# atom501/v-img

Measured on AMD Instinct MI355X. Metric: Mrays/sec (primary+secondary) at 512 spp, higher is better.
Workload: dtype f32; 1 GPU; disney_spheres.json, mis integrator, 512 spp, 1800x800; integrator=mis, spp=512, depth=unbounded, bvh=sweep SAH (host)

## Files before the change

v-img_amd/csrc/device_scene.h:

```cpp
#pragma once
#include <hip/hip_runtime.h>
#include <stdint.h>

#include "../../include/vimg_scene.h"
#include "material_record.h"

namespace vimg {

#define VIMG_GLOBAL __attribute__((address_space(1)))
#define VIMG_LDS __attribute__((address_space(3)))
template <typename T>
using gptr = const VIMG_GLOBAL T*;
typedef float v4f __attribute__((ext_vector_type(4)));
typedef uint32_t v2u __attribute__((ext_vector_type(2)));
typedef uint32_t v4u __attribute__((ext_vector_type(4)));

struct __attribute__((aligned(16))) DNode {
  v4f a;
  v4f b;
  v4f c;
  uint32_t left_ref, right_ref, pad0, pad1;
};
static_assert(sizeof(DNode) == 64, "DNode must be one 64-byte line");

// ... 61 lines not shown
};

struct RenderArgs {
  uint32_t integrator, samples, depth;
  uint32_t tile_rank, tile_world;
  uint32_t tiles_x, tiles_y;
  uint32_t num_local_tiles;
  uint32_t full_stats;
  uint32_t stack_entries;
  uint32_t lds_nodes;
  uint32_t stack_lds;
  VIMG_GLOBAL uint32_t* stack_ovf;
  VIMG_GLOBAL v4u* pool_cold;
  uint32_t lds_leaf;
  VIMG_GLOBAL v4u* pool_state;
  uint32_t pool_segments;
  uint32_t pool_seg_len;
  uint32_t pool_epoch;
  uint32_t pool_slots;
  uint32_t pool_refill;
  uint32_t pool_vbatch;
  uint32_t pool_boxmin;
  uint32_t pool_starve;
  uint32_t pool_gbreak;
  uint32_t pool_classes;
  uint32_t cu_walkers;
  uint32_t cu_flex;
  uint32_t cu_lowwater;
  uint32_t cu_patience;
  uint32_t cu_join;
  uint32_t cu_sleep;
  uint32_t cu_watchdog;
  uint32_t cu_magic_v, cu_shift_v;
  uint32_t cu_magic_w, cu_shift_w;
  int32_t single_x, single_y;
  uint32_t sample_base;
  float spp_div;
  const VIMG_GLOBAL v4u* prog_in;
  VIMG_GLOBAL v4u* prog_out;
  const VIMG_GLOBAL uint32_t* item_list;
  uint32_t item_count;
};

struct DeviceStats {
  unsigned long long closest, shadow, internal, leaf, prim, sphere, nan_samples;
  unsigned long long trip_descend, trip_prim, iterations;
  unsigned long long prof[28];
  unsigned long long wait_cyc[5], wait_n[5];
  unsigned long long px_done[3];
  unsigned long long px_hops[3];
  unsigned long long ray_cyc[2];
  unsigned long long pv_cyc[7];
  unsigned long long walk_cyc[4];
};

}
```

v-img_amd/csrc/render_cu_kernel.h:

```cpp
#pragma once
#include <type_traits>

#include "plain_build.h"
#include "render_kernels.h"

namespace vimg {

enum : uint32_t {
  SC_THROUGHPUT = 0,
  SC_RESULT,
  SC_NEE,
  SC4_RNG,
  SC4_MAIN
};
__host__ __device__ constexpr uint32_t cu_cold_records(bool tex) { return SC4_MAIN + 1u + (tex ? 1u : 0u); }
__host__ __device__ constexpr uint32_t cu_stack_rows_of(uint32_t entries, uint32_t in_lds) { return in_lds < entries ? in_lds + 1u : entries; }
constexpr uint32_t SLOT_IDLE = 0xffffffffu;

VD void state_store(VIMG_GLOBAL uint32_t* p, uint32_t v) {
  __hip_atomic_store(p, v, __ATOMIC_RELAXED, __HIP_MEMORY_SCOPE_AGENT);
}
VD uint32_t state_load(VIMG_GLOBAL uint32_t* p) {
  return __hip_atomic_load(p, __ATOMIC_RELAXED, __HIP_MEMORY_SCOPE_AGENT);
}
VD uint32_t lane_rank(unsigned long long mask, uint32_t lane) {
  return __popcll(mask & ((1ull << lane) - 1ull));
}

enum : uint32_t {
  CF_PRIMARY = 1u, CF_NONSPEC = 2u, CF_HAS_S = 4u, CF_HAS_R = 8u, CF_OCCLUDED = 16u, CF_FOUND = 32u,
  CF_FRESH = 64u, CF_KIND_SPHERE = 128u, CF_DONE_S = 256u, CF_DONE_R = 512u,
  CF_CLS_SHIFT = 10u,
  CF_DONE_V = 4096u,
  CF_KILL_R = 8192u,
  CF_BOUNCE_SHIFT = 16u
};
enum : uint32_t {
  CR_ORG = 0,
  CR_DIR,
  CR_SHD,
  CR_HIT,
  CR_COUNT
};
constexpr uint32_t CU_EMPTY = 0xffffu;
constexpr uint32_t CU_RAY_S = 0x8000u;
constexpr uint32_t CQ_WALK = 4u, CQ_COUNT = 5u;
constexpr uint32_t CU_LDS_BYTES = CR_COUNT * 16u + 8u + 4u * 2u + 2u * 2u + 4u;

struct CuCtl {
  int32_t avail[8];
  uint32_t tail[CQ_COUNT], head[CQ_COUNT];
  uint32_t live;
  uint32_t pixels_left;
  uint32_t abort;
  uint32_t t0_lo, t0_hi;
  uint32_t pad[1];
};
static_assert(sizeof(CuCtl) == 96, "CuCtl layout");
struct CuWaveRec {
  unsigned long long cyc[6], nbatch[4], nslots[4];
  uint32_t internal, leaf, prim, sphere;
  unsigned long long box_pass, box_lanes, leaf_round, leaf_lanes, sessions, refills, refill_rays, pad;
  unsigned long long looks, q_sum[4];
  unsigned long long w_cyc[4];
  unsigned long long wait_cyc[5], wait_n[5];
  unsigned long long ray_cyc, ray_n;
  unsigned long long pv_cyc[6], pv_n;
};
static_assert(sizeof(CuWaveRec) == 416, "CuWaveRec layout");
__host__ __device__ constexpr uint32_t cu_pool_bytes(uint32_t slots, uint32_t waves) {
  return CU_LDS_BYTES * slots + uint32_t(sizeof(CuCtl)) + waves * uint32_t(sizeof(CuWaveRec));
}
VD uint32_t cu_mod(uint32_t n, uint32_t d, uint32_t magic, uint32_t shift) { return n - d * (__umulhi(n, magic) >> shift); }
VD int32_t lds_add_rtn(VIMG_LDS int32_t* p, int32_t v) { return __hip_atomic_fetch_add(p, v, __ATOMIC_RELAXED, __HIP_MEMORY_SCOPE_WORKGROUP); }
VD uint32_t lds_add_rtn(VIMG_LDS uint32_t* p, uint32_t v) { return __hip_atomic_fetch_add(p, v, __ATOMIC_RELAXED, __HIP_MEMORY_SCOPE_WORKGROUP); }
VD uint32_t lds_load(VIMG_LDS uint32_t* p) { return __hip_atomic_load(p, __ATOMIC_RELAXED, __HIP_MEMORY_SCOPE_WORKGROUP); }
VD int32_t lds_load(VIMG_LDS int32_t* p) { return __hip_atomic_load(p, __ATOMIC_RELAXED, __HIP_MEMORY_SCOPE_WORKGROUP); }
VD uint32_t cu_uni(uint32_t v) { return static_cast<uint32_t>(__builtin_amdgcn_readfirstlane(static_cast<int>(v))); }

static_assert(PLAIN_INTEGRATOR_MIS == uint32_t(VIMG_INTEGRATOR_MIS), "plain_build.h");
template <uint32_t PLAIN> VD uint32_t opt_integrator(const RenderArgs& A) {
  if constexpr (PLAIN & PF_INTEGRATOR) return uint32_t(VIMG_INTEGRATOR_MIS); else return A.integrator;
}
template <uint32_t PLAIN> VD uint32_t opt_classes(const RenderArgs& A) {
  if constexpr (PLAIN & PF_CLASSES) return 3u; else return A.pool_classes;
}
template <uint32_t PLAIN> VD bool opt_leaf_in_lds(const RenderArgs& A) {
  if constexpr (PLAIN & PF_LEAF_LDS) return true; else return A.lds_leaf != 0u;
}
template <uint32_t PLAIN> VD bool opt_single(const RenderArgs& A) {
  if constexpr (PLAIN & PF_SINGLE) return false; else return A.single_x >= 0;
}
template <uint32_t PLAIN> VD bool opt_has_items(const RenderArgs& A) {
  if constexpr (PLAIN & PF_ITEMS) return false; else return A.item_list != nullptr;
}
template <uint32_t PLAIN> VD uint32_t opt_flex(const RenderArgs& A) {
  if constexpr (PLAIN & PF_FLEX) return PLAIN_FLEX_DEFAULT; else return A.cu_flex;
}


struct CuKArgs {
  DScene g;
  RenderArgs A;
  float* out;
  DeviceStats* stats;
  unsigned int* work_counter;
};
typedef const __attribute__((address_space(4))) CuKArgs* CuKPtr;
VD CuKPtr cu_kargs() {
  unsigned long long p = reinterpret_cast<unsigned long long>(__builtin_amdgcn_kernarg_segment_ptr());
  asm volatile("" : "+s"(p));
  return (CuKPtr)p;
}

#define CU_STAGE_LOCALS(K)                                                                                              \
  extern __shared__ __attribute__((aligned(16))) unsigned char lds_raw[];                                               \
  [[maybe_unused]] const DScene& g = *(const DScene*)&(K)->g;                                                           \
  [[maybe_unused]] const RenderArgs& A = *(const RenderArgs*)&(K)->A;                                                   \
  [[maybe_unused]] float* __restrict__ out = (K)->out;                                                                  \
  [[maybe_unused]] unsigned int* __restrict__ work_counter = (K)->work_counter;                                         \
// ... 133 lines not shown
        VIMG_LDS uint16_t* e_ = ring_at(q, h_ + r_);                                                                    \
        uint32_t v_ = __hip_atomic_load(e_, __ATOMIC_RELAXED, __HIP_MEMORY_SCOPE_WORKGROUP), spins_ = 0;                \
        while (v_ == CU_EMPTY && !stuck_) {                                                                             \
          __builtin_amdgcn_s_sleep(1);                                                                                  \
          v_ = __hip_atomic_load(e_, __ATOMIC_RELAXED, __HIP_MEMORY_SCOPE_WORKGROUP);                                   \
          if (++spins_ > (1u << 22)) stuck_ = true;                                                                     \
        }                                                                                                               \
        __hip_atomic_store(e_, static_cast<uint16_t>(CU_EMPTY), __ATOMIC_RELAXED, __HIP_MEMORY_SCOPE_WORKGROUP);        \
        entry = v_;                                                                                                     \
      }                                                                                                                 \
    }                                                                                                                   \
    if (__any(stuck_)) {                                                                                                \
      if (lane == 0) raise(4u);                                                                                         \
      return 0u;                                                                                                        \
    }                                                                                                                   \
    return got_;                                                                                                        \
  }

template <bool TEX, int NW, bool DIAG, int EARLY, bool FIN, int MTC, uint32_t PLAIN>
VD void cu_vertex(uint32_t n, uint32_t slot, bool& all_pending, uint32_t& n_nan, uint32_t& n_dead) {
  const CuKPtr K = cu_kargs();
  CU_STAGE_LOCALS(K);
  constexpr bool finisher_batch = FIN;
  constexpr bool CAN_SPLIT = !FIN && MTC != int(VIMG_MAT_LAMBERTIAN);
  const bool split = CAN_SPLIT && n <= 32u && !(opt_flex<PLAIN>(A) & 16u);
  const bool mirror = split && lane >= 32u;
  if (split) slot = static_cast<uint32_t>(__shfl(static_cast<int>(slot), static_cast<int>(lane & 31u)));
  const bool on = (split ? (lane & 31u) : lane) < n;
  if (!on) slot = 0u;
  const v4u r_ray = on ? rd(CR_DIR, slot) : v4u{0u, 0u, 0u, 0u};
  uint32_t flags = r_ray.w;
  const bool fresh = on && (flags & CF_FRESH);
  const bool have = on && !fresh;
  uint32_t px = 0, py = 0, smp = 0, item = 0, bounce = 0;
  Rng rng{0};
  f3 acc{0.f, 0.f, 0.f}, ray_o{0.f, 0.f, 0.f}, ray_d{0.f, 0.f, 1.f};
  f3 throughput{1.f, 1.f, 1.f}, result{0.f, 0.f, 0.f};
  RayCone cone{0.f, 0.f};
  float eta_scale = 1.f, prev_pdf = 0.f;
  bool primary = true, non_specular_bounce = false;
  v4u r_origin{0u, 0u, 0u, 0u}, r_hit{0u, 0u, 0u, 0u}, r_nee{0u, 0u, 0u, 0u};
  v2u r_hx{0u, 0u};
  constexpr bool PV = DIAG && MTC == int(VIMG_MAT_PRINCIPLED);
  [[maybe_unused]] unsigned long long pv_t = PV ? __builtin_readcyclecounter() : 0ull;
  [[maybe_unused]] auto pv_lap = [&](int k) {
    if constexpr (PV) {
      if (full_stats) {
        const unsigned long long now = __builtin_readcyclecounter();
        if (lane == 0) wrec->pv_cyc[k] += now - pv_t;
        pv_t = now;
      }
    }
  };
  uint32_t hops = 0;
  if (full_stats && have) hops = recw[(CR_SHD * P + slot) * 4u + 3u] + 1u;
  if (have) {
    const v4u r_t = crd(SC_THROUGHPUT, slot), r_r = crd(SC_RESULT, slot);
    v4u r_a{0u, 0u, 0u, 0u};
    if (finisher_batch) r_a = cold_acc[slot];
    if (r_ray.w & CF_HAS_S) r_nee = crd(SC_NEE, slot);
    r_origin = rd(CR_ORG, slot);
    r_hit = rd(CR_HIT, slot);
    r_hx = hitx[slot];
    const v4u r_g = crd(SC4_RNG, slot);
    px = r_g.z & 0xffffu, py = r_g.z >> 16;
    smp = r_g.w;
    item = r_a.w;
    rng.s = uint64_t(r_g.x) | (uint64_t(r_g.y) << 32);
    acc = f3{uf(r_a.x), uf(r_a.y), uf(r_a.z)};
    ray_o = f3{uf(r_origin.x), uf(r_origin.y), uf(r_origin.z)};
    ray_d = f3{uf(r_ray.x), uf(r_ray.y), uf(r_ray.z)};
    throughput = f3{uf(r_t.x), uf(r_t.y), uf(r_t.z)};
    result = f3{uf(r_r.x), uf(r_r.y), uf(r_r.z)};
    eta_scale = uf(r_t.w);
    prev_pdf = uf(r_r.w);
    bounce = flags >> CF_BOUNCE_SHIFT;
    primary = (flags & CF_PRIMARY) != 0;
    non_specular_bounce = (flags & CF_NONSPEC) != 0;
    if constexpr (TEX) {
      const v4u r_c = cold_cone[slot];
      cone = RayCone{uf(r_c.x), uf(r_c.y)};
    }
  }

  pv_lap(0);
  bool finish = false, at_vertex = false;
  Hit hit;
  hit.p = f3{0.f, 0.f, 0.f};
  if (have) {
    if ((flags & CF_HAS_S) && !(flags & CF_OCCLUDED))
      result = result + f3{uf(r_nee.x), uf(r_nee.y), uf(r_nee.z)};
    if (!(flags & CF_HAS_R) || (flags & CF_KILL_R)) {
      finish = true;
    } else {
      const bool hit_any = (flags & CF_FOUND) != 0;
      if (hit_any) {
        HitRec hr;
        hr.e0 = uf(r_hit.x), hr.e1 = uf(r_hit.y), hr.e2 = uf(r_hit.z);
        hr.inv_det = uf(r_hit.w);
        hr.prim = r_hx.x;
        hr.kind = (flags & CF_KIND_SPHERE) ? 1u : 0u;
        TravRay tr{ray_o, ray_d, 0.0001f, uf(r_hx.y)};
        make_hit_info<TEX>(g, hr, tr, hit);
      }
      if (material_mode) {
        if (!hit_any) {
          result = throughput * background_emit<TEX>(g, ray_d, cone);
          finish = true;
        } else {
          at_vertex = true;
// ... 22 lines not shown
            at_vertex = true;
          }
        }
      } else {
        if (hit_any) {
          gptr<VimgMaterial> m = g.materials + hit.mat;
          if (m->type == VIMG_MAT_DIFFUSE_LIGHT) {
            const f3 le = mat_emitted(m, ray_d, hit.ns);
            if (prev_pdf != 0) {
              float light_pdf = surf_pdf(g, hit.prim, ray_o, hit.p, ray_d) / g.num_lights;
              float Gt = geometric_term(ray_o, hit.p, hit.ng);
              float mis_weight = balance_heuristic(prev_pdf * Gt, light_pdf);
              result = result + throughput * mis_weight * le;
            } else {
              result = result + throughput * le;
            }
            finish = true;
          } else {
            bool survive = true;
            if (bounce > roulette_threshold) {
              float rr = static_cast<float>(pcg_next(rng)) / 4294967296.0f;
              f3 rr_t = (1.f / eta_scale) * throughput;
              float max_val = sel_min(sel_max(sel_max(rr_t.x, rr_t.y), rr_t.z), 0.95f);
              if (rr > max_val)
                survive = false;
              else
                throughput = throughput / max_val;
            }
            if (survive) {
              bounce += 1;
              at_vertex = true;
            } else {
              finish = true;
            }
          }
        } else {
          if (prev_pdf != 0 && g.background_emissive) {
            float light_pdf = background_pdf<TEX>(g, ray_d) / g.num_lights;
            float mis_weight = balance_heuristic(prev_pdf, light_pdf);
            result = result + throughput * mis_weight * background_emit<TEX>(g, ray_d, cone);
          }
          finish = true;
        }
      }
      if (at_vertex && !(bounce < A.depth)) {
        at_vertex = false;
        finish = true;
      }
    }
  }

  pv_lap(1);
  if constexpr (!finisher_batch) {
    if (have && !mirror) {
      VIMG_GLOBAL uint32_t* rw = reinterpret_cast<VIMG_GLOBAL uint32_t*>(cold + (slot * SC4_MAIN + SC_RESULT));
      rw[0] = fu(result.x), rw[1] = fu(result.y), rw[2] = fu(result.z);
    }
  }
  bool has_s = false, has_r = false;
  bool early = false, pushed_r = false;
  bool rec_written = false;
  f3 shadow_d{0.f, 0.f, 1.f}, nee_contrib{0.f, 0.f, 0.f};
  float shadow_max_t = 0.f;
  if constexpr (!finisher_batch) {
    if (material_mode && at_vertex) {
      gptr<VimgMaterial> m = g.materials + hit.mat;
      const f3 emitted_col = mat_emitted(m, ray_d, hit.ns);
      Scatter sc = sample_mat<TEX>(g, hit, ray_d, rng, non_specular_bounce);
      if (!sc.valid) {
        result = throughput * emitted_col;
        finish = true;
      } else {
        if (!sc.is_specular) non_specular_bounce = true;
        if constexpr (TEX) {
          const float hd = length(ray_o - hit.p);
          const float ssa = spread_angle_from_curvature(hit.curvature, cone.cone_width, ray_d, hit.ns);
          if (sc.eta != 0.f)
            cone = propagate_refract_cone(cone, ray_d, ssa, sc.eta, sc.wo);
          else
            cone = propagate_reflect_cone(cone, ssa * 2.f, hd);
        }
        if (sc.eta != 0.f) eta_scale /= (sc.eta * sc.eta);
        f3 fdiv{0.f, 0.f, 0.f};
        const uint32_t type = m->type;
        if (type == VIMG_MAT_LAMBERTIAN) {
          fdiv = col_at_ray_hit<TEX>(g, m->tex, ray_d, cone, hit);
        } else if (type == VIMG_MAT_DIELECTRIC) {
          fdiv = splat3(1.f);
        } else if (type == VIMG_MAT_PRINCIPLED) {
          f3 f;
          float pdf;
          principled_eval_pdf<TEX>(g, m, ray_d, sc.wo, hit, cone, non_specular_bounce, f, pdf);
          fdiv = f / pdf;
        }
        throughput = throughput * (emitted_col + fdiv);
        bool survive = true;
        if (bounce > roulette_threshold) {
          float rr = static_cast<float>(pcg_next(rng)) / 4294967296.0f;
          f3 rr_t = (1.f / eta_scale) * throughput;
          float max_val = sel_min(sel_max(sel_max(rr_t.x, rr_t.y), rr_t.z), 0.95f);
          if (rr > max_val)
            survive = false;
          else
            throughput = throughput / max_val;
        }
        bounce += 1;
// ... 204 lines not shown
          }
          if (!valid) {
            have_claim = false;
          } else if (seg == 0u) {
            if (A.sample_base == 0u) {
              const uint64_t image_index = uint64_t(px) + uint64_t(H - 1 - py) * W;
              pcg_seed(rng, image_index);
              acc = f3{0.f, 0.f, 0.f};
            } else {
              const v4u r0 = A.prog_in[size_t(item) * 2u], r1 = A.prog_in[size_t(item) * 2u + 1u];
              rng.s = uint64_t(r0.x) | (uint64_t(r0.y) << 32);
              acc = f3{uf(r1.x), uf(r1.y), uf(r1.z)};
            }
            smp = 0;
            need_pixel = false;
          } else {
            VIMG_GLOBAL uint32_t* st = reinterpret_cast<VIMG_GLOBAL uint32_t*>(A.pool_state + size_t(item) * 2u);
            const uint32_t done = state_load(st + 2);
            if (done == A.pool_epoch + seg) {
              __builtin_amdgcn_fence(__ATOMIC_ACQUIRE, "workgroup");
              const uint32_t r_lo = state_load(st + 0), r_hi = state_load(st + 1);
              rng.s = uint64_t(r_lo) | (uint64_t(r_hi) << 32);
              acc = f3{uf(state_load(st + 4)), uf(state_load(st + 5)), uf(state_load(st + 6))};
              smp = seg * seg_len;
              need_pixel = false;
            } else {
              pending = true;
            }
          }
        }
      }
    }
    n_nan += static_cast<uint32_t>(__popcll(__ballot(is_nan_sample)));
    all_pending = (__ballot(pending) == __ballot(on));
    const bool regen = on && !retire && !pending && (finish || fresh);
    if (regen) {
      const f2 off = random_x_y_r2(px + py + A.sample_base + smp);
      const float rand2 = rand_float(rng);
      const float rand1 = rand_float(rng);
      generate_ray(g, static_cast<float>(px) + off.x, static_cast<float>(py) + off.y, rand1, rand2, ray_o, ray_d);
      cone = RayCone{0.f, g.cone_spread};
      throughput = f3{1.f, 1.f, 1.f};
      result = f3{0.f, 0.f, 0.f};
      eta_scale = 1.f;
      non_specular_bounce = false;
      primary = true;
      bounce = 0;
      has_s = false;
      has_r = true;
    }
  }

  const bool keep = on && !retire && !mirror;
  if (keep) {
    if (!early) {
      const uint32_t nf = pending ? (CF_FRESH | CF_PRIMARY)
                                  : ((primary ? CF_PRIMARY : 0u) | (non_specular_bounce ? CF_NONSPEC : 0u) |
                                     (has_s ? CF_HAS_S : 0u) | (has_r ? CF_HAS_R : 0u) | CF_DONE_V | (bounce << CF_BOUNCE_SHIFT));
      if (pending) has_s = false, has_r = false, smp = claim;
      if (rec_written) {
        *flag_word(slot) = nf;
      } else {
        wr(CR_ORG, slot, v4u{fu(ray_o.x), fu(ray_o.y), fu(ray_o.z), fu(shadow_max_t)});
        wr(CR_DIR, slot, v4u{fu(ray_d.x), fu(ray_d.y), fu(ray_d.z), nf});
        if (has_s) wr(CR_SHD, slot, v4u{fu(shadow_d.x), fu(shadow_d.y), fu(shadow_d.z), hops});
        else if (full_stats) recw[(CR_SHD * P + slot) * 4u + 3u] = hops;
      }
    }
    cwr(SC_THROUGHPUT, slot, v4u{fu(throughput.x), fu(throughput.y), fu(throughput.z), fu(eta_scale)});
    if constexpr (finisher_batch) {
      cwr(SC_RESULT, slot, v4u{fu(result.x), fu(result.y), fu(result.z), fu(prev_pdf)});
      cwr(SC4_RNG, slot, v4u{static_cast<uint32_t>(rng.s), static_cast<uint32_t>(rng.s >> 32), px | (py << 16), smp});
    } else {
      VIMG_GLOBAL uint32_t* rw = reinterpret_cast<VIMG_GLOBAL uint32_t*>(cold + (slot * SC4_MAIN + SC_RESULT));
      rw[3] = fu(prev_pdf);
      if (material_mode) rw[0] = fu(result.x), rw[1] = fu(result.y), rw[2] = fu(result.z);
      *reinterpret_cast<VIMG_GLOBAL v2u*>(cold + (slot * SC4_MAIN + SC4_RNG)) = v2u{static_cast<uint32_t>(rng.s), static_cast<uint32_t>(rng.s >> 32)};
    }
    if (has_s) cwr(SC_NEE, slot, v4u{fu(nee_contrib.x), fu(nee_contrib.y), fu(nee_contrib.z), 0u});
    if (finisher_batch) cold_acc[slot] = v4u{fu(acc.x), fu(acc.y), fu(acc.z), item};
    if constexpr (TEX) cold_cone[slot] = v4u{fu(cone.cone_width), fu(cone.spread_angle), 0u, 0u};
  }
  if (full_stats && keep && !early) tq[slot] = static_cast<uint32_t>(__builtin_readcyclecounter());
  __builtin_amdgcn_s_waitcnt(0x0F70);
  {
    push_rays(keep && !early && has_s, keep && !early && has_r, slot);
    push(0u, __ballot(keep && !early && !has_s && !has_r), slot);
    const uint32_t n_retired = static_cast<uint32_t>(__popcll(__ballot(on && retire)));
    if (n_retired && lane == 0) __hip_atomic_fetch_sub(&G->live, n_retired, __ATOMIC_RELAXED, __HIP_MEMORY_SCOPE_WORKGROUP);
  }
  if constexpr (!FIN) {
    if (EARLY == 2 ? (cu_uni(A.cu_flex) & 32u) != 0u : (EARLY == 1)) {
      const bool mine = keep && early, dead = mine && pushed_r && !has_r;
      uint32_t nw = 0;
      bool complete = false;
      if (mine) {
        const uint32_t orv = CF_DONE_V | (dead ? CF_KILL_R : 0u);
        nw = __hip_atomic_fetch_or(flag_word(slot), orv, __ATOMIC_ACQ_REL, __HIP_MEMORY_SCOPE_WORKGROUP) | orv;
        complete = slot_complete(nw);
      }
      hand_to_vertex(complete, nw, slot);
      n_dead += static_cast<uint32_t>(__popcll(__ballot(dead)));
    }
  }
  pv_lap(5);
  if constexpr (PV) {
    if (full_stats && lane == 0) wrec->pv_n += 1;
  }
}

template <bool TEX, bool DEEP, int NW, bool DIAG, uint32_t PLAIN>
VD void cu_walk(uint32_t& n_closest, uint32_t& n_shadow) {
  const CuKPtr K = cu_kargs();
  CU_STAGE_LOCALS(K);
  const Lds L = lds_layout(A, (VIMG_LDS unsigned char*)lds_raw);
  const uint32_t S = A.stack_lds;
  VIMG_GLOBAL uint32_t* ovf0 = A.stack_ovf + (size_t(blockIdx.x) * A.cu_walkers + (can_walk ? wave : 0u)) * ((A.stack_entries - S) * 64u) + lane;
  uint32_t w_slot = SLOT_IDLE, w_type = 0, w_cls = 0, sp = 0, cur = REF_DONE;
  bool w_setup = false, w_any = false, w_found = false, w_exact = false;
  TravRay ray{f3{0.f, 0.f, 0.f}, f3{0.f, 0.f, 1.f}, 0.0001f, VIMG_INF};
  f3 w_inv{1.f, 1.f, 1.f};
  TriRayConst rc{0.f, 0.f, 1.f, 2};
  float w_dir_len2 = 1.f;
  HitRec rec;
  rec.prim = 0xffffffffu, rec.kind = 0;
  rec.e0 = rec.e1 = rec.e2 = rec.inv_det = 0.f;
  uint32_t c_internal = 0, c_leaf = 0, c_prim = 0, c_sphere = 0;
  uint32_t d_box = 0, d_boxl = 0, d_leaf = 0, d_leafl = 0, d_ref = 0, d_refr = 0;
  uint32_t t_in = 0;
  unsigned long long d_waitc = 0, d_rayc = 0;
  uint32_t d_waitn = 0, d_rayn = 0;
  unsigned long long wt = full_stats ? __builtin_readcyclecounter() : 0ull, wc0 = 0, wc1 = 0, wc2 = 0, wc3 = 0;
  auto wlap = [&](unsigned long long& acc) {
    if (full_stats) {
      const unsigned long long now = __builtin_readcyclecounter();
      acc += now - wt;
      wt = now;
    }
  };
  for (;;) {
    {
      const unsigned long long m_idle = __ballot(w_slot == SLOT_IDLE);
      const uint32_t n_idle = static_cast<uint32_t>(__popcll(m_idle));
      if (n_idle >= A.pool_refill || n_idle == 64u) {
        const int32_t aw = static_cast<int32_t>(cu_uni(static_cast<uint32_t>(lds_load(&G->avail[CQ_WALK]))));
        if (aw > 0) {
          const uint32_t want = n_idle < static_cast<uint32_t>(aw) ? n_idle : static_cast<uint32_t>(aw);
          uint32_t e = 0;
          const uint32_t got = pop(CQ_WALK, want, m_idle, e);
          d_ref += stat_inc, d_refr += full_stats ? got : 0u;
          if (w_slot == SLOT_IDLE && lane_rank(m_idle, lane) < got) {
            if (full_stats) {
              t_in = static_cast<uint32_t>(__builtin_readcyclecounter());
              d_waitc += static_cast<unsigned long long>(t_in - tq[e & 0x7fffu]), d_waitn += 1u;
            }
            w_slot = e & 0x7fffu;
            w_type = (e & CU_RAY_S) ? 0u : 1u;
// ... 128 lines not shown
        const uint32_t sp_below = sp != 0 ? sp - 1 : 0u;
        uint32_t popped = stack0[(DEEP ? (sp_below < S ? sp_below : S) : sp_below) * 64];
        if constexpr (DEEP) {
          if (!stop && sp_below >= S) popped = ovf0[(sp_below - S) * 64];
        }
        cur = (stop || sp == 0) ? REF_DONE : popped;
        sp = sp_below;
      }
      wlap(wc2);
      const uint32_t n_fin = static_cast<uint32_t>(__popcll(__ballot(w_slot != SLOT_IDLE && cur == REF_DONE)));
      const uint32_t n_act = static_cast<uint32_t>(__popcll(__ballot(w_slot != SLOT_IDLE && cur != REF_DONE)));
      if (n_act == 0 || n_fin >= A.pool_refill) break;
    }

    {
      const bool done = w_slot != SLOT_IDLE && cur == REF_DONE;
      bool complete = false;
      uint32_t nw = 0;
      if (done) {
        uint32_t orv;
        if (w_type == 0u) {
          orv = CF_DONE_S | (w_found ? CF_OCCLUDED : 0u);
        } else {
          orv = CF_DONE_R;
          if (w_found) {
            orv |= CF_FOUND | (rec.kind == 1 ? CF_KIND_SPHERE : 0u) | (w_cls << CF_CLS_SHIFT);
            wr(CR_HIT, w_slot, v4u{fu(rec.e0), fu(rec.e1), fu(rec.e2), fu(rec.inv_det)});
            hitx[w_slot] = v2u{rec.prim, fu(ray.max_t)};
          }
        }
        nw = __hip_atomic_fetch_or(flag_word(w_slot), orv, __ATOMIC_ACQ_REL, __HIP_MEMORY_SCOPE_WORKGROUP) | orv;
        complete = slot_complete(nw);
      }
      if (__any(done)) {
        hand_to_vertex(complete, nw, w_slot);
        if (full_stats && done) d_rayc += static_cast<unsigned long long>(static_cast<uint32_t>(__builtin_readcyclecounter()) - t_in), d_rayn += 1u;
        if (done) w_slot = SLOT_IDLE;
      }
    }
    wlap(wc3);
    if (cu_uni(lds_load(&G->abort)) != 0u) break;
  }
  if (full_stats) {
    if (lane == 0) wrec->w_cyc[0] += wc0, wrec->w_cyc[1] += wc1, wrec->w_cyc[2] += wc2, wrec->w_cyc[3] += wc3;
    auto wsum = [](unsigned long long v) {
      for (int o = 32; o; o >>= 1) v += __shfl_xor(v, o);
      return v;
    };
    const unsigned long long s_int = wsum(c_internal), s_leaf = wsum(c_leaf), s_prim = wsum(c_prim), s_sph = wsum(c_sphere);
    const unsigned long long s_wc = wsum(d_waitc), s_wn = wsum(d_waitn), s_rc = wsum(d_rayc), s_rn = wsum(d_rayn);
    if (lane == 0) {
      wrec->internal += static_cast<uint32_t>(s_int), wrec->leaf += static_cast<uint32_t>(s_leaf);
      wrec->prim += static_cast<uint32_t>(s_prim), wrec->sphere += static_cast<uint32_t>(s_sph);
      wrec->wait_cyc[4] += s_wc, wrec->wait_n[4] += s_wn, wrec->ray_cyc += s_rc, wrec->ray_n += s_rn;
    }
    if (lane == 0) {
      wrec->box_pass += d_box, wrec->box_lanes += d_boxl, wrec->leaf_round += d_leaf, wrec->leaf_lanes += d_leafl;
      wrec->sessions += 1, wrec->refills += d_ref, wrec->refill_rays += d_refr;
    }
  }
}

template <bool TEX, bool DEEP, int NW, int WPS, bool DIAG, int EARLY, uint32_t PLAIN = 0u>
__global__ void __launch_bounds__(NW * 64, WPS)
render_cu_kernel(const CuKArgs ka) {
  {
    const CuKPtr K = cu_kargs();
    CU_STAGE_LOCALS(K);
    stage_lds(g, A, (VIMG_LDS unsigned char*)lds_raw);
    for (uint32_t i = lane; i < sizeof(CuWaveRec) / 4u; i += 64u) reinterpret_cast<VIMG_LDS uint32_t*>(wrec)[i] = 0u;
    for (uint32_t i = threadIdx.x; i < A.lds_leaf * 3u; i += blockDim.x)
      lds_leaf[i] = reinterpret_cast<gptr<v4f>>(g.leaf_prims)[i];
    for (uint32_t s = threadIdx.x; s < P; s += blockDim.x) {
      recw[(CR_DIR * P + s) * 4u + 3u] = CF_FRESH;
      ring_v[s] = static_cast<uint16_t>(s);
      ring_v[P + s] = CU_EMPTY, ring_v[2u * P + s] = CU_EMPTY, ring_v[3u * P + s] = CU_EMPTY;
      ring_w[s] = CU_EMPTY, ring_w[P + s] = CU_EMPTY;
      tq[s] = static_cast<uint32_t>(__builtin_readcyclecounter());
    }
    if (threadIdx.x == 0) {
      for (uint32_t q = 0; q < 8u; ++q) G->avail[q] = (q == 0u) ? static_cast<int32_t>(P) : 0;
      G->live = P, G->pixels_left = 1u, G->abort = 0u;
      for (uint32_t q = 0; q < CQ_COUNT; ++q) G->tail[q] = (q == 0u) ? P : 0u, G->head[q] = 0u;
      const unsigned long long t0 = __builtin_amdgcn_s_memrealtime();
      G->t0_lo = static_cast<uint32_t>(t0), G->t0_hi = static_cast<uint32_t>(t0 >> 32);
    }
    __syncthreads();
  }
  uint32_t n_closest = 0, n_shadow = 0, n_nan = 0, iter_wave = 0;
  uint32_t n_dead = 0;
  unsigned long long t_mark = __builtin_readcyclecounter();
  bool skip_fin = false;
  uint32_t polls = 0;
  unsigned long long idle_since = 0;
  for (;;) {
    const CuKPtr K = cu_kargs();
    CU_STAGE_LOCALS(K);
    auto lap = [&](uint32_t k) {
      if (full_stats) {
        const unsigned long long now = __builtin_readcyclecounter();
        if (lane == 0) wrec->cyc[k] += now - t_mark;
        t_mark = now;
      }
    };
    if (cu_uni(lds_load(&G->abort)) != 0u) break;
    const v4u av4 = *reinterpret_cast<VIMG_LDS v4u*>(&G->avail[0]);
    const int32_t a0 = skip_fin ? 0 : static_cast<int32_t>(cu_uni(av4.x)), a1 = static_cast<int32_t>(cu_uni(av4.y)),
// ... 34 lines not shown
        if (lane == 0) wrec->wait_cyc[cls] += w, wrec->wait_n[cls] += n;
      }
      bool all_pending = false;
      const bool by_class = opt_classes<PLAIN>(A) == 3u;
      if (opt_flex<PLAIN>(A) & 2u) __builtin_amdgcn_s_setprio(1);
      if (cls == 0u)
        cu_vertex<TEX, NW, DIAG, EARLY, true, -1, PLAIN>(n, e, all_pending, n_nan, n_dead);
      else if (cls == 1u && by_class)
        cu_vertex<TEX, NW, DIAG, EARLY, false, int(VIMG_MAT_LAMBERTIAN), PLAIN>(n, e, all_pending, n_nan, n_dead);
      else if (cls == 2u && by_class)
        cu_vertex<TEX, NW, DIAG, EARLY, false, int(VIMG_MAT_PRINCIPLED), PLAIN>(n, e, all_pending, n_nan, n_dead);
      else
        cu_vertex<TEX, NW, DIAG, EARLY, false, -1, PLAIN>(n, e, all_pending, n_nan, n_dead);
      if (opt_flex<PLAIN>(A) & 2u) __builtin_amdgcn_s_setprio(0);
      skip_fin = all_pending;
      if (!all_pending) polls = 0, idle_since = 0;
      lap(cls);
      continue;
    }
    if (cu_uni(lds_load(&G->live)) == 0u) break;
    skip_fin = false;
    polls += 1;
    if ((polls & 255u) == 0u) {
      const unsigned long long now = __builtin_amdgcn_s_memrealtime();
      if (idle_since == 0) idle_since = now;
      else if (static_cast<uint32_t>((now - idle_since) >> 20) > A.cu_watchdog) {
        if (lane == 0) raise(1u);
        break;
      }
    }
    if (A.cu_sleep >= 32u) __builtin_amdgcn_s_sleep(32);
    else if (A.cu_sleep >= 16u) __builtin_amdgcn_s_sleep(16);
    else if (A.cu_sleep >= 8u) __builtin_amdgcn_s_sleep(8);
    else if (A.cu_sleep >= 4u) __builtin_amdgcn_s_sleep(4);
    else __builtin_amdgcn_s_sleep(1);
  }

  {
    const CuKPtr K = cu_kargs();
    CU_STAGE_LOCALS(K);
    DeviceStats* __restrict__ stats = K->stats;
    if (full_stats && lane == 0) wrec->cyc[5] += __builtin_readcyclecounter() - t_mark;
    if (stats && lane == 0) {
      atomicAdd(&stats->closest, static_cast<unsigned long long>(n_closest) - static_cast<unsigned long long>(n_dead));
      atomicAdd(&stats->shadow, static_cast<unsigned long long>(n_shadow));
      if (n_nan) atomicAdd(&stats->nan_samples, static_cast<unsigned long long>(n_nan));
      if (full_stats) {
        atomicAdd(&stats->internal, static_cast<unsigned long long>(wrec->internal));
        atomicAdd(&stats->leaf, static_cast<unsigned long long>(wrec->leaf));
        atomicAdd(&stats->prim, static_cast<unsigned long long>(wrec->prim));
        atomicAdd(&stats->sphere, static_cast<unsigned long long>(wrec->sphere));
        atomicAdd(&stats->iterations, static_cast<unsigned long long>(iter_wave));
        for (int k = 0; k < 6; ++k) atomicAdd(&stats->prof[k], wrec->cyc[k]);
        for (int k = 0; k < 4; ++k) atomicAdd(&stats->prof[6 + k], wrec->nbatch[k]), atomicAdd(&stats->prof[11 + k], wrec->nslots[k]);
        atomicAdd(&stats->prof[10], 1ull);
        const unsigned long long wd[7] = {wrec->box_pass, wrec->box_lanes, wrec->leaf_round, wrec->leaf_lanes, wrec->sessions,
                                          wrec->refills, wrec->refill_rays};
        for (int k = 0; k < 7; ++k) atomicAdd(&stats->prof[16 + k], wd[k]);
        atomicAdd(&stats->prof[23], wrec->looks);
        for (int k = 0; k < 4; ++k) atomicAdd(&stats->prof[24 + k], wrec->q_sum[k]);
        for (int k = 0; k < 4; ++k) atomicAdd(&stats->walk_cyc[k], wrec->w_cyc[k]);
        for (int k = 0; k < 5; ++k) atomicAdd(&stats->wait_cyc[k], wrec->wait_cyc[k]), atomicAdd(&stats->wait_n[k], wrec->wait_n[k]);
        atomicAdd(&stats->ray_cyc[0], wrec->ray_cyc), atomicAdd(&stats->ray_cyc[1], wrec->ray_n);
        for (int k = 0; k < 6; ++k) atomicAdd(&stats->pv_cyc[k], wrec->pv_cyc[k]);
        atomicAdd(&stats->pv_cyc[6], wrec->pv_n);
      }
    }
  }
}

}
```

v-img_amd/csrc/vimg_hip.hip:

```cpp
#include <cstdio>
#include <cstdlib>
#include <memory>

#include "hip_internal.h"
#include "aux_kernels.h"
#include "render_cu_kernel.h"
#include "heatmap_kernel.h"

namespace vimg {

hipStream_t g_stream = nullptr;
int g_device = -1;

namespace {
thread_local std::string g_err;
}

int fail(int code, const std::string& msg) {
  g_err = msg;
  return code;
}

}

// ... 106 lines not shown
}

uint64_t fetch_shard_pixels(const VimgDeviceScene* s, const VimgRenderParams* p) {
  const uint32_t W = s->d.res_x, H = s->d.res_y, ty_n = tiles_of(H), total = tiles_of(W) * ty_n;
  uint64_t px = 0;
  for (uint32_t t = p->tile_rank; t < total; t += p->tile_world) {
    uint32_t tx = t / ty_n, ty = t % ty_n;
    px += uint64_t(std::min(8u, W - tx * 8)) * std::min(8u, H - ty * 8);
  }
  return px;
}

int fetch_stats(VimgDeviceScene* s, const VimgRenderParams* p, VimgRenderStats* out) {
  DeviceStats ds{};
  HIP_TRY(hipMemcpy(&ds, s->stats.p, sizeof(ds), hipMemcpyDeviceToHost));
  *out = VimgRenderStats{};
  out->closest_rays = ds.closest;
  out->shadow_rays = ds.shadow;
  out->internal_visits = ds.internal;
  out->leaf_visits = ds.leaf;
  out->prim_tests = ds.prim;
  out->sphere_tests = ds.sphere;
  out->nan_samples = ds.nan_samples;
  out->paths = fetch_shard_pixels(s, p) * p->samples;
  if (getenv("VIMG_HIP_DIAG"))
    std::fprintf(stderr, "[vimg diag] wave trips: descend %llu (lane visits %llu, util %.3f)  prim %llu (lane tests %llu, util %.3f)  main-loop iterations %llu\n",
                 ds.trip_descend, ds.internal, ds.trip_descend ? double(ds.internal) / (64.0 * ds.trip_descend) : 0.0,
                 ds.trip_prim, ds.prim, ds.trip_prim ? double(ds.prim) / (64.0 * ds.trip_prim) : 0.0, ds.iterations);
  if (getenv("VIMG_HIP_DIAG") && ds.prof[6 + 4]) {
    static const char* st_names[6] = {"finisher", "lambertian", "principled", "other", "walk", "looking for work"};
    unsigned long long total = 0;
    for (int k = 0; k < 6; ++k) total += ds.prof[k];
    for (int k = 0; k < 6; ++k)
      std::fprintf(stderr, "[vimg stage] %-18s %14llu cyc %6.2f %%  batches %10llu  slots/batch %7.2f\n", st_names[k],
                   ds.prof[k], 100.0 * double(ds.prof[k]) / double(total ? total : 1), k < 5 ? ds.prof[6 + k] : 0ull,
                   (k < 5 && ds.prof[6 + k]) ? double(ds.prof[11 + k]) / double(ds.prof[6 + k]) : 0.0);
    if (ds.prof[16])
      std::fprintf(stderr, "[vimg walk] box passes %llu lanes/pass %.2f   leaf rounds %llu lanes/round %.2f   sessions %llu   refills %llu rays/refill %.2f\n",
                   ds.prof[16], double(ds.prof[17]) / double(ds.prof[16]), ds.prof[18], double(ds.prof[19]) / double(ds.prof[18] ? ds.prof[18] : 1),
                   ds.prof[20], ds.prof[21], double(ds.prof[22]) / double(ds.prof[21] ? ds.prof[21] : 1));
    if (ds.wait_n[4])
      std::fprintf(stderr, "[vimg wait] mean cycles in a ring before a wave takes the slot: finisher %.0f  lambertian %.0f  principled %.0f  other %.0f  walk %.0f\n",
                   double(ds.wait_cyc[0]) / double(ds.wait_n[0] ? ds.wait_n[0] : 1), double(ds.wait_cyc[1]) / double(ds.wait_n[1] ? ds.wait_n[1] : 1),
                   double(ds.wait_cyc[2]) / double(ds.wait_n[2] ? ds.wait_n[2] : 1), double(ds.wait_cyc[3]) / double(ds.wait_n[3] ? ds.wait_n[3] : 1),
                   double(ds.wait_cyc[4]) / double(ds.wait_n[4]));
    if (ds.ray_cyc[1])
      std::fprintf(stderr, "[vimg wait] mean cycles of a ray in a walking lane (pop to hand-over) %.0f; of a vertex batch: finisher %.0f lambertian %.0f principled %.0f other %.0f\n",
                   double(ds.ray_cyc[0]) / double(ds.ray_cyc[1]), double(ds.prof[0]) / double(ds.prof[6] ? ds.prof[6] : 1), double(ds.prof[1]) / double(ds.prof[7] ? ds.prof[7] : 1),
                   double(ds.prof[2]) / double(ds.prof[8] ? ds.prof[8] : 1), double(ds.prof[3]) / double(ds.prof[9] ? ds.prof[9] : 1));
    if (ds.pv_cyc[6])
      std::fprintf(stderr, "[vimg wait] a Principled batch, mean cycles: state loads %.0f  hit record + path logic %.0f  light sample %.0f  BSDF sample %.0f  evaluations %.0f  stores + hand-over %.0f\n",
                   double(ds.pv_cyc[0]) / double(ds.pv_cyc[6]), double(ds.pv_cyc[1]) / double(ds.pv_cyc[6]), double(ds.pv_cyc[2]) / double(ds.pv_cyc[6]),
                   double(ds.pv_cyc[3]) / double(ds.pv_cyc[6]), double(ds.pv_cyc[4]) / double(ds.pv_cyc[6]), double(ds.pv_cyc[5]) / double(ds.pv_cyc[6]));
    if (ds.px_done[1])
      std::fprintf(stderr, "[vimg wait] pixels finished (last sample written) after: mean %.3f ms, latest %.3f ms\n",
                   double(ds.px_done[0]) / double(ds.px_done[1]) * 1e-5, double(ds.px_done[2]) * 1e-5);
    if (ds.px_done[1])
      std::fprintf(stderr, "[vimg wait] vertex-stage visits per pixel: mean %.1f, most %llu; the pixel that finished last: %llu visits in %.3f ms = %.2f us per visit (walks included)\n",
                   double(ds.px_hops[0]) / double(ds.px_done[1]), ds.px_hops[1], ds.px_hops[2] & 0xffffffull, double(ds.px_hops[2] >> 24) * 1e-5,
                   double(ds.px_hops[2] >> 24) * 1e-2 / double((ds.px_hops[2] & 0xffffffull) ? (ds.px_hops[2] & 0xffffffull) : 1));
    if (ds.prof[23])
      std::fprintf(stderr, "[vimg walk] cycles: refill+setup %llu  box %llu  leaf %llu  hand-over %llu   |  looks %llu  mean ring counts seen: finisher %.1f lambertian %.1f principled %.1f walk %.1f\n",
                   ds.walk_cyc[0], ds.walk_cyc[1], ds.walk_cyc[2], ds.walk_cyc[3], ds.prof[23], double(ds.prof[24]) / double(ds.prof[23]),
                   double(ds.prof[25]) / double(ds.prof[23]), double(ds.prof[26]) / double(ds.prof[23]), double(ds.prof[27]) / double(ds.prof[23]));
#ifdef VIMG_WALK_DIAG
    static const char* wd_names[12] = {"walk: refill+setup cyc", "walk: box loop cyc", "walk: leaf rounds cyc", "walk: retire cyc",
                                       "box trips", "box lanes", "leaf rounds", "leaf lanes", "leaf prim trips",
                                       "retire: cyc to get lock", "retire: cyc to unlock", "retire: lock takes"};
    for (int k = 0; k < 12; ++k) std::fprintf(stderr, "[vimg walk] %-24s %14llu\n", wd_names[k], ds.prof[16 + k]);
#endif
  }
  return VIMG_OK;
}

}

extern "C" {

const char* vimg_hip_last_error(void) { return g_err.c_str(); }

int vimg_hip_device_count(void) {
  int n = 0;
  hipError_t e = hipGetDeviceCount(&n);
  if (e != hipSuccess) return fail(VIMG_E_DEVICE, std::string("hipGetDeviceCount: ") + hipGetErrorString(e));
  return n;
}

int vimg_hip_init(int device_ordinal) {
  HIP_TRY(hipSetDevice(device_ordinal));
  if (!g_stream) HIP_TRY(hipStreamCreateWithFlags(&g_stream, hipStreamNonBlocking));
  g_device = device_ordinal;
  return VIMG_OK;
}

void vimg_hip_options_default(VimgHipOptions* o) {
  if (!o) return;
  int32_t* f = reinterpret_cast<int32_t*>(o);
  for (size_t i = 1; i < sizeof(VimgHipOptions) / sizeof(int32_t); ++i) f[i] = VIMG_OPT_AUTO;
  o->struct_size = sizeof(VimgHipOptions);
}

int64_t vimg_hip_shard_pixels(const VimgDeviceScene* s, const VimgRenderParams* p) {
  int rc = check_params(s, p);
  if (rc) return rc;
  return int64_t(local_tiles(s, p)) * 64;
}
// ... 175 lines not shown
```

Measured before the change: 15170 Mrays/s.

## Replace full waitcnt before ray pushes with workgroup release fence and skip camera-ray state loads

Moves the vmcnt wait that preceded the hand-over pushes to sit before the cold-state stores, and after those stores uses a workgroup release fence plus an acquire fence at batch start. The intent is to stop each wave from blocking on the completion of its own global stores before publishing slots. Camera rays now skip loading throughput and result records and use constants instead. The finisher no longer writes throughput and result records. It also adds tail-cycle diagnostics and shrinks some counters to 32 bits. The new memory-ordering scheme risks visibility bugs if the fences do not cover the cross-wave handoff.

```diff
diff --git a/v-img_amd/csrc/device_scene.h b/v-img_amd/csrc/device_scene.h
--- a/v-img_amd/csrc/device_scene.h
+++ b/v-img_amd/csrc/device_scene.h
@@ -137,6 +137,7 @@
   unsigned long long ray_cyc[2];
   unsigned long long pv_cyc[7];
   unsigned long long walk_cyc[4];
+  unsigned long long tail_cyc[3][2];
 };
 
 }
diff --git a/v-img_amd/csrc/render_cu_kernel.h b/v-img_amd/csrc/render_cu_kernel.h
--- a/v-img_amd/csrc/render_cu_kernel.h
+++ b/v-img_amd/csrc/render_cu_kernel.h
@@ -58,14 +58,17 @@
 };
 static_assert(sizeof(CuCtl) == 96, "CuCtl layout");
 struct CuWaveRec {
-  unsigned long long cyc[6], nbatch[4], nslots[4];
+  unsigned long long cyc[6];
+  uint32_t nbatch[4], nslots[4];
   uint32_t internal, leaf, prim, sphere;
   unsigned long long box_pass, box_lanes, leaf_round, leaf_lanes, sessions, refills, refill_rays, pad;
   unsigned long long looks, q_sum[4];
   unsigned long long w_cyc[4];
-  unsigned long long wait_cyc[5], wait_n[5];
+  unsigned long long wait_cyc[5];
+  uint32_t wait_n[5], pad2;
   unsigned long long ray_cyc, ray_n;
   unsigned long long pv_cyc[6], pv_n;
+  unsigned long long tail_cyc[3][2];
 };
 static_assert(sizeof(CuWaveRec) == 416, "CuWaveRec layout");
 __host__ __device__ constexpr uint32_t cu_pool_bytes(uint32_t slots, uint32_t waves) {
@@ -305,10 +308,24 @@
       }
     }
   };
+  constexpr int TAIL_CLS = FIN ? 0 : (MTC == int(VIMG_MAT_LAMBERTIAN) ? 1 : (MTC == int(VIMG_MAT_PRINCIPLED) ? 2 : -1));
+  [[maybe_unused]] unsigned long long tail_t = 0ull;
+  [[maybe_unused]] auto tail_lap = [&](int k) {
+    if constexpr (DIAG && TAIL_CLS >= 0) {
+      if (full_stats) {
+        const unsigned long long now = __builtin_readcyclecounter();
+        if (k >= 0 && lane == 0) wrec->tail_cyc[TAIL_CLS][k] += now - tail_t;
+        tail_t = now;
+      }
+    }
+  };
   uint32_t hops = 0;
   if (full_stats && have) hops = recw[(CR_SHD * P + slot) * 4u + 3u] + 1u;
+  __builtin_amdgcn_fence(__ATOMIC_ACQUIRE, "workgroup");
   if (have) {
-    const v4u r_t = crd(SC_THROUGHPUT, slot), r_r = crd(SC_RESULT, slot);
+    const bool camera = (flags & (CF_PRIMARY | CF_HAS_R)) == (CF_PRIMARY | CF_HAS_R);
+    v4u r_t{fu(1.f), fu(1.f), fu(1.f), fu(1.f)}, r_r{0u, 0u, 0u, 0u};
+    if (!camera) r_t = crd(SC_THROUGHPUT, slot), r_r = crd(SC_RESULT, slot);
     v4u r_a{0u, 0u, 0u, 0u};
     if (finisher_batch) r_a = cold_acc[slot];
     if (r_ray.w & CF_HAS_S) r_nee = crd(SC_NEE, slot);
@@ -437,6 +454,7 @@
 
   pv_lap(1);
   if constexpr (!finisher_batch) {
+    __builtin_amdgcn_s_waitcnt(0x0F70);
     if (have && !mirror) {
       VIMG_GLOBAL uint32_t* rw = reinterpret_cast<VIMG_GLOBAL uint32_t*>(cold + (slot * SC4_MAIN + SC_RESULT));
       rw[0] = fu(result.x), rw[1] = fu(result.y), rw[2] = fu(result.z);
@@ -747,6 +765,7 @@
   }
 
   const bool keep = on && !retire && !mirror;
+  __builtin_amdgcn_s_waitcnt(0x0F70);
   if (keep) {
     if (!early) {
       const uint32_t nf = pending ? (CF_FRESH | CF_PRIMARY)
@@ -762,11 +781,10 @@
         else if (full_stats) recw[(CR_SHD * P + slot) * 4u + 3u] = hops;
       }
     }
-    cwr(SC_THROUGHPUT, slot, v4u{fu(throughput.x), fu(throughput.y), fu(throughput.z), fu(eta_scale)});
     if constexpr (finisher_batch) {
-      cwr(SC_RESULT, slot, v4u{fu(result.x), fu(result.y), fu(result.z), fu(prev_pdf)});
       cwr(SC4_RNG, slot, v4u{static_cast<uint32_t>(rng.s), static_cast<uint32_t>(rng.s >> 32), px | (py << 16), smp});
     } else {
+      cwr(SC_THROUGHPUT, slot, v4u{fu(throughput.x), fu(throughput.y), fu(throughput.z), fu(eta_scale)});
       VIMG_GLOBAL uint32_t* rw = reinterpret_cast<VIMG_GLOBAL uint32_t*>(cold + (slot * SC4_MAIN + SC_RESULT));
       rw[3] = fu(prev_pdf);
       if (material_mode) rw[0] = fu(result.x), rw[1] = fu(result.y), rw[2] = fu(result.z);
@@ -777,7 +795,9 @@
     if constexpr (TEX) cold_cone[slot] = v4u{fu(cone.cone_width), fu(cone.spread_angle), 0u, 0u};
   }
   if (full_stats && keep && !early) tq[slot] = static_cast<uint32_t>(__builtin_readcyclecounter());
-  __builtin_amdgcn_s_waitcnt(0x0F70);
+  tail_lap(-1);
+  __builtin_amdgcn_fence(__ATOMIC_RELEASE, "workgroup");
+  tail_lap(0);
   {
     push_rays(keep && !early && has_s, keep && !early && has_r, slot);
     push(0u, __ballot(keep && !early && !has_s && !has_r), slot);
@@ -798,6 +818,7 @@
       n_dead += static_cast<uint32_t>(__popcll(__ballot(dead)));
     }
   }
+  tail_lap(1);
   pv_lap(5);
   if constexpr (PV) {
     if (full_stats && lane == 0) wrec->pv_n += 1;
@@ -1032,7 +1053,7 @@
     if (lane == 0) {
       wrec->internal += static_cast<uint32_t>(s_int), wrec->leaf += static_cast<uint32_t>(s_leaf);
       wrec->prim += static_cast<uint32_t>(s_prim), wrec->sphere += static_cast<uint32_t>(s_sph);
-      wrec->wait_cyc[4] += s_wc, wrec->wait_n[4] += s_wn, wrec->ray_cyc += s_rc, wrec->ray_n += s_rn;
+      wrec->wait_cyc[4] += s_wc, wrec->wait_n[4] += static_cast<uint32_t>(s_wn), wrec->ray_cyc += s_rc, wrec->ray_n += s_rn;
     }
     if (lane == 0) {
       wrec->box_pass += d_box, wrec->box_lanes += d_boxl, wrec->leaf_round += d_leaf, wrec->leaf_lanes += d_leafl;
@@ -1173,7 +1194,7 @@
         atomicAdd(&stats->sphere, static_cast<unsigned long long>(wrec->sphere));
         atomicAdd(&stats->iterations, static_cast<unsigned long long>(iter_wave));
         for (int k = 0; k < 6; ++k) atomicAdd(&stats->prof[k], wrec->cyc[k]);
-        for (int k = 0; k < 4; ++k) atomicAdd(&stats->prof[6 + k], wrec->nbatch[k]), atomicAdd(&stats->prof[11 + k], wrec->nslots[k]);
+        for (int k = 0; k < 4; ++k) atomicAdd(&stats->prof[6 + k], static_cast<unsigned long long>(wrec->nbatch[k])), atomicAdd(&stats->prof[11 + k], static_cast<unsigned long long>(wrec->nslots[k]));
         atomicAdd(&stats->prof[10], 1ull);
         const unsigned long long wd[7] = {wrec->box_pass, wrec->box_lanes, wrec->leaf_round, wrec->leaf_lanes, wrec->sessions,
                                           wrec->refills, wrec->refill_rays};
@@ -1181,13 +1202,14 @@
         atomicAdd(&stats->prof[23], wrec->looks);
         for (int k = 0; k < 4; ++k) atomicAdd(&stats->prof[24 + k], wrec->q_sum[k]);
         for (int k = 0; k < 4; ++k) atomicAdd(&stats->walk_cyc[k], wrec->w_cyc[k]);
-        for (int k = 0; k < 5; ++k) atomicAdd(&stats->wait_cyc[k], wrec->wait_cyc[k]), atomicAdd(&stats->wait_n[k], wrec->wait_n[k]);
+        for (int k = 0; k < 5; ++k) atomicAdd(&stats->wait_cyc[k], wrec->wait_cyc[k]), atomicAdd(&stats->wait_n[k], static_cast<unsigned long long>(wrec->wait_n[k]));
         atomicAdd(&stats->ray_cyc[0], wrec->ray_cyc), atomicAdd(&stats->ray_cyc[1], wrec->ray_n);
         for (int k = 0; k < 6; ++k) atomicAdd(&stats->pv_cyc[k], wrec->pv_cyc[k]);
         atomicAdd(&stats->pv_cyc[6], wrec->pv_n);
-      }
-    }
-  }
-}
-
-}
+        for (int k = 0; k < 3; ++k) atomicAdd(&stats->tail_cyc[k][0], wrec->tail_cyc[k][0]), atomicAdd(&stats->tail_cyc[k][1], wrec->tail_cyc[k][1]);
+      }
+    }
+  }
+}
+
+}
diff --git a/v-img_amd/csrc/vimg_hip.hip b/v-img_amd/csrc/vimg_hip.hip
--- a/v-img_amd/csrc/vimg_hip.hip
+++ b/v-img_amd/csrc/vimg_hip.hip
@@ -182,6 +182,10 @@
       std::fprintf(stderr, "[vimg wait] a Principled batch, mean cycles: state loads %.0f  hit record + path logic %.0f  light sample %.0f  BSDF sample %.0f  evaluations %.0f  stores + hand-over %.0f\n",
                    double(ds.pv_cyc[0]) / double(ds.pv_cyc[6]), double(ds.pv_cyc[1]) / double(ds.pv_cyc[6]), double(ds.pv_cyc[2]) / double(ds.pv_cyc[6]),
                    double(ds.pv_cyc[3]) / double(ds.pv_cyc[6]), double(ds.pv_cyc[4]) / double(ds.pv_cyc[6]), double(ds.pv_cyc[5]) / double(ds.pv_cyc[6]));
+    if (ds.prof[6] && ds.prof[7] && ds.prof[8])
+      std::fprintf(stderr, "[vimg wait] tail of a batch, mean cycles (last cold store to the end of the wait | pushes): finisher %.0f | %.0f  lambertian %.0f | %.0f  principled %.0f | %.0f\n",
+                   double(ds.tail_cyc[0][0]) / double(ds.prof[6]), double(ds.tail_cyc[0][1]) / double(ds.prof[6]), double(ds.tail_cyc[1][0]) / double(ds.prof[7]),
+                   double(ds.tail_cyc[1][1]) / double(ds.prof[7]), double(ds.tail_cyc[2][0]) / double(ds.prof[8]), double(ds.tail_cyc[2][1]) / double(ds.prof[8]));
     if (ds.px_done[1])
       std::fprintf(stderr, "[vimg wait] pixels finished (last sample written) after: mean %.3f ms, latest %.3f ms\n",
                    double(ds.px_done[0]) / double(ds.px_done[1]) * 1e-5, double(ds.px_done[2]) * 1e-5);
```

Result: no change. 15310 Mrays/s, median of 6 (+0.9%).
